# twosixlabs/csl-gan

Measured on AMD Instinct MI355X. Metric: images/sec/GPU CelebA DCResNet dp_mode=gc bs=128 at 1/2/4/8 MI355X, higher is better.
Workload: dtype f32; 1 GPU; CelebA DCResNet D-step: dp_mode=gc -gcm adaptive-pl -nms 32, WGAN-GP on mean samples, 3x64x64; compute_dtype=fp32_auto, storage_dtype=fp32, launch=hip_graph, batch_per_gpu=128, global_batch=128, parallelism=dp1, materialize=ghost, grad_sample_dtype=fp32, fuse_passes=True

## Files before the change

csl_gan_amd/csrc/igemm_x3.hip:

```cpp
#include <stdlib.h>
#include "common.h"
#include "igemm.h"

namespace cslgan {

typedef float f32x16 __attribute__((ext_vector_type(16)));
typedef float f32x2 __attribute__((ext_vector_type(2)));
typedef __bf16 bf16x2 __attribute__((ext_vector_type(2)));
typedef __bf16 bf16x8 __attribute__((ext_vector_type(8)));
typedef unsigned int u32x4 __attribute__((ext_vector_type(4)));

namespace {

constexpr unsigned XOOB = 0xFFFFFFF0u;
constexpr unsigned XFAR = 0xFFFF0000u;
constexpr int XH_MAX = 160;
constexpr int XROW = 12, XQROW = 6, XQIMG = 40;

__device__ __forceinline__ unsigned xpack(float lo, float hi) {
    const f32x2 v = {lo, hi};
    return __builtin_bit_cast(unsigned, __builtin_convertvector(v, bf16x2));
}
__device__ __forceinline__ float xlo(unsigned u) { return __uint_as_float(u << 16); }
__device__ __forceinline__ float xhi(unsigned u) { return __uint_as_float(u & 0xffff0000u); }
struct x3_t { uint2 hi, mid, lo; };
__device__ __forceinline__ x3_t xsplit4(const float4& v) {
    x3_t r;
    r.hi = make_uint2(xpack(v.x, v.y), xpack(v.z, v.w));
    const float r0 = v.x - xlo(r.hi.x), r1 = v.y - xhi(r.hi.x), r2 = v.z - xlo(r.hi.y), r3 = v.w - xhi(r.hi.y);
    r.mid = make_uint2(xpack(r0, r1), xpack(r2, r3));
    r.lo = make_uint2(xpack(r0 - xlo(r.mid.x), r1 - xhi(r.mid.x)), xpack(r2 - xlo(r.mid.y), r3 - xhi(r.mid.y)));
    return r;
}
__device__ __forceinline__ float4 xload4(__amdgpu_buffer_rsrc_t r, unsigned byte_off) {
    const u32x4 v = __builtin_amdgcn_raw_buffer_load_b128(r, (int)byte_off, 0, 0);
    return make_float4(__uint_as_float(v.x), __uint_as_float(v.y), __uint_as_float(v.z), __uint_as_float(v.w));
}

}

template <int BN, int NP, bool GEN, bool AFF = false>
__global__ __launch_bounds__(256, 2) void igemm_x3h_kernel(const KcParams p) {
    constexpr int BM = 128, TM = 2, TN = BN / 64;
    constexpr bool F32 = NP == 0;
    constexpr int NI = F32 ? 1 : NP;
    constexpr int NO = F32 ? 2 : NP;
    constexpr int PXU = F32 ? 4 : 2;
    constexpr int IMG = 2 * XH_MAX * PXU;
    __shared__ __attribute__((aligned(16))) uint4 Hs[2][NI][IMG];
    __shared__ int s_off[BM];
    __shared__ int s_roff[BM];

    const int tid = threadIdx.x;
    const int nwg = p.tiles_m * p.tiles_n;
    const int cs = p.csplit > 1 ? p.csplit : 1;
    const int wgs = xcd_remap(blockIdx.x, nwg * cs);
    const int split = cs > 1 ? wgs % cs : 0;
    const int wg = cs > 1 ? wgs / cs : wgs;
    const int tile_mg = wg / p.tiles_n, tile_n = wg - tile_mg * p.tiles_n;
    const bool accumulate = GEN && p.acc_classes;
    const int n_sub = accumulate ? p.n_cls : ((GEN && p.pair_mode) ? 2 : 1);
    const int lane = tid & 63, wid = tid >> 6;
    const int r = lane & 31, h = lane >> 5;
    const int wm = wid >> 1, wn = wid & 1;
    const int n0 = tile_n * BN;
    const __amdgpu_buffer_rsrc_t a_rsrc = __builtin_amdgcn_make_buffer_rsrc(const_cast<float*>(p.a), 0, p.a_bytes, 0x00020000);

    f32x16 acc[TM][TN];
#pragma unroll 1
    for (int sub = 0; sub < n_sub; ++sub) {
        int ci = 0, tile_in_cls;
        if (accumulate) {
            ci = sub;
            tile_in_cls = tile_mg;
        } else if (GEN && p.pair_mode) {
            const int pg = tile_mg / p.tiles_per_cls;
            ci = p.pair_cls[pg][sub];
            tile_in_cls = tile_mg - pg * p.tiles_per_cls;
        } else {
            if (GEN) {
#pragma unroll 1
                while (ci + 1 < p.n_cls && tile_mg >= p.cls[ci + 1].tile0) ++ci;
            }
            tile_in_cls = tile_mg - p.cls[ci].tile0;
        }
        const KcClass& kc = p.cls[ci];
        const int M = kc.M, OHc = kc.OHc, OWc = kc.OWc, T = kc.T;
        const int m0 = tile_in_cls * BM;
        const int HW_ = kc.halo_w, HH_ = kc.halo_h;
        const bool quad = GEN && kc.patch == 2;
        const int hpix_img = HH_ * HW_;
        const int hpix = quad ? 4 * hpix_img : hpix_img;
        const int img_stride = p.AH * p.AW * p.AC;
        const int ay_mul = (GEN && kc.ay_mul) ? kc.ay_mul : 1, ay_off = GEN ? kc.ay_off : 0;
        const int ax_mul = (GEN && kc.ax_mul) ? kc.ax_mul : 1, ax_off = GEN ? kc.ax_off : 0;
        const int nkw = kc.nkw;
        const int ystep = T > nkw ? (int)kc.ty[nkw] - (int)kc.ty[0] : 0;
        const int xstep = nkw > 1 ? (int)kc.tx[1] - (int)kc.tx[0] : 0;
        const int dy0 = (int)kc.ty[0] - kc.ty_min, dx0 = (int)kc.tx[0] - kc.tx_min;

        constexpr int HREG = (2 * XH_MAX * 4 + 255) / 256;
        unsigned h_goff[HREG];
        int h_lds[HREG];
        unsigned pp_mask = 0;
        int aff_off[2] = {0, 0};
        {
            int p_img[2], p_y0[2], p_x0[2];
            bool p_ok[2];
#pragma unroll
            for (int pp = 0; pp < 2; ++pp) {
                const int m = m0 + 64 * pp;
                p_ok[pp] = m < M;
                const RowCoord rc = kc_decode_row(p_ok[pp] ? m : 0, OHc, OWc, quad ? 0 : 1);
                p_img[pp] = rc.img * img_stride;
                if (AFF) aff_off[pp] = rc.img * p.AC + (tid & 3) * 4;
                p_y0[pp] = rc.oy + kc.ty_min;
                p_x0[pp] = rc.ox + kc.tx_min;
            }
            const int h_total = 2 * hpix * 4;
#pragma unroll
            for (int j = 0; j < HREG; ++j) {
                const int idx = tid + 256 * j;
                const int ch = idx & 3, pixg = idx >> 2;
                const int pp = pixg >= hpix ? 1 : 0;
                pp_mask |= (unsigned)pp << j;
                const int pix = pixg - pp * hpix;
                const int si = quad ? pix / hpix_img : 0;
                const int rem = pix - si * hpix_img;
                const int hy = rem / HW_, hx = rem - hy * HW_;
                const int iy = (p_y0[pp] + hy) * ay_mul + ay_off, ix = (p_x0[pp] + hx) * ax_mul + ax_off;
                const bool in_img = idx < h_total && p_ok[pp] && (unsigned)iy < (unsigned)p.VH && (unsigned)ix < (unsigned)p.VW;
                h_goff[j] = in_img ? 4u * (unsigned)(p_img[pp] + si * img_stride + (iy * p.AW + ix) * p.AC + ch * 4) : XFAR;
                const int lpx = quad ? si * XQIMG + hy * XQROW + hx : hy * XROW + hx;
                h_lds[j] = idx >= h_total ? -1 : (F32 ? (pp * XH_MAX + lpx) * 4 + (ch ^ ((hx + hy) & 3)) : (pp * XH_MAX + lpx) * 4 + (ch ^ ((hy & 1) << 1)));
            }
        }
        const int n_cc_all = p.AC >> 4;
        const int cc_lo = cs > 1 ? split * n_cc_all / cs : 0;
        const int n_cc = cs > 1 ? (split + 1) * n_cc_all / cs - cc_lo : n_cc_all;
        const float lo = (AFF && !p.in_relu) ? -__builtin_inff() : 0.f;
        float4 rh[HREG];
        float4 sc0, sc1, sh0, sh1;
        const __amdgpu_buffer_rsrc_t sc_rsrc = __builtin_amdgcn_make_buffer_rsrc(const_cast<float*>(AFF ? p.in_scale : p.a), 0, 0xFFFFFFF0u, 0x00020000);
        const __amdgpu_buffer_rsrc_t sh_rsrc = __builtin_amdgcn_make_buffer_rsrc(const_cast<float*>(AFF ? p.in_shift : p.a), 0, 0xFFFFFFF0u, 0x00020000);
        auto fetch_halo = [&](int cc) {
            const unsigned co = 64u * (unsigned)(cc + cc_lo);
#pragma unroll
            for (int j = 0; j < HREG; ++j) rh[j] = xload4(a_rsrc, h_goff[j] + co);
            if (AFF) {
                sc0 = xload4(sc_rsrc, 4u * (unsigned)aff_off[0] + co); sh0 = xload4(sh_rsrc, 4u * (unsigned)aff_off[0] + co);
                sc1 = xload4(sc_rsrc, 4u * (unsigned)aff_off[1] + co); sh1 = xload4(sh_rsrc, 4u * (unsigned)aff_off[1] + co);
            }
        };
        auto commit_halo = [&](int buf) {
#pragma unroll
            for (int j = 0; j < HREG; ++j) {
                if (AFF) {
                    const bool second = (pp_mask >> j) & 1u;
                    const float m = h_goff[j] != XFAR ? 1.f : 0.f;
                    rh[j].x = fmaxf(fmaf((second ? sc1.x : sc0.x) * m, rh[j].x, (second ? sh1.x : sh0.x) * m), lo);
                    rh[j].y = fmaxf(fmaf((second ? sc1.y : sc0.y) * m, rh[j].y, (second ? sh1.y : sh0.y) * m), lo);
                    rh[j].z = fmaxf(fmaf((second ? sc1.z : sc0.z) * m, rh[j].z, (second ? sh1.z : sh0.z) * m), lo);
                    rh[j].w = fmaxf(fmaf((second ? sc1.w : sc0.w) * m, rh[j].w, (second ? sh1.w : sh0.w) * m), lo);
                }
                if (h_lds[j] >= 0) {
                    uint2* img0 = reinterpret_cast<uint2*>(&Hs[buf][0][0]);
                    if (F32) {
                        Hs[buf][0][h_lds[j]] = make_uint4(__float_as_uint(rh[j].x), __float_as_uint(rh[j].y), __float_as_uint(rh[j].z), __float_as_uint(rh[j].w));
                    } else if (NP == 1) {
                        img0[h_lds[j]] = make_uint2(xpack(rh[j].x, rh[j].y), xpack(rh[j].z, rh[j].w));
                    } else {
                        const x3_t t3 = xsplit4(rh[j]);
                        img0[h_lds[j]] = t3.hi;
                        reinterpret_cast<uint2*>(&Hs[buf][NI > 1 ? 1 : 0][0])[h_lds[j]] = t3.mid;
                        reinterpret_cast<uint2*>(&Hs[buf][NI > 2 ? 2 : 0][0])[h_lds[j]] = t3.lo;
                    }
                }
            }
        };

        const unsigned piece_bytes = F32 ? 32u : 2u * (unsigned)p.Nn * (unsigned)kc.Kdim;
        const __amdgpu_buffer_rsrc_t w3_rsrc = __builtin_amdgcn_make_buffer_rsrc(
            const_cast<char*>(reinterpret_cast<const char*>(p.w3) + (F32 ? 4ll : 2ll * NP) * kc.w_off), 0,
            F32 ? 4u * (unsigned)p.Nn * (unsigned)kc.Kdim : NP * piece_bytes, 0x00020000);
        const unsigned n_bytes = F32 ? 64u : 32u;
        const unsigned step_bytes = n_bytes * (unsigned)p.Nn;
        unsigned b_off[TN];
#pragma unroll
        for (int j = 0; j < TN; ++j) {
            const int n = n0 + wn * TN * 32 + j * 32 + r;
            b_off[j] = n < p.Nn ? n_bytes * (unsigned)n + 16u * (unsigned)h : XOOB;
        }
        const int n_steps = n_cc * T;
        const unsigned step0_bytes = (unsigned)(cc_lo * T) * step_bytes;
        u32x4 B0[NO][TN], B1[NO][TN];
        auto load_b = [&](int step, u32x4 (&dst)[NO][TN]) {
            const unsigned kb = (unsigned)step * step_bytes + step0_bytes;
            const unsigned past = step >= n_steps ? XOOB : 0u;
#pragma unroll
            for (int j = 0; j < TN; ++j) {
                const unsigned bad = past | (b_off[j] == XOOB ? XOOB : 0u);
#pragma unroll
                for (int c = 0; c < NO; ++c)
                    dst[c][j] = __builtin_amdgcn_raw_buffer_load_b128(w3_rsrc, (int)((b_off[j] + kb + c * piece_bytes) | bad), 0, 0);
            }
        };

        int a_idx[TM];
        int a_rot[TM];
#pragma unroll
        for (int i = 0; i < TM; ++i) {
            const int qq = i * 32 + r;
            const int ly = quad ? (qq >> 2) & 3 : qq >> 3;
            const int lx = quad ? qq & 3 : qq & 7;
            const int lpix = quad ? (qq >> 4) * XQIMG + ly * XQROW + lx : ly * XROW + lx;
            a_idx[i] = F32 ? (wm * XH_MAX + lpix) * 4 : (wm * XH_MAX + lpix) * 2 + (h ^ (ly & 1));
            a_rot[i] = (lx + ly) & 3;
        }
        const int HWL = quad ? XQROW : XROW;
        u32x4 A0[NO][TM], A1[NO][TM];
        auto read_a = [&](int buf, int dy, int dx, u32x4 (&dst)[NO][TM]) {
            const int poff = dy * HWL + dx;
#pragma unroll
            for (int i = 0; i < TM; ++i) {
                if (F32) {
                    const int rot = (a_rot[i] + dy + dx) & 3, base = a_idx[i] + 4 * poff;
#pragma unroll
                    for (int c = 0; c < NO; ++c) {
                        const uint4 v = Hs[buf][0][base + ((2 * c + h) ^ rot)];
                        dst[c][i] = u32x4{v.x, v.y, v.z, v.w};
                    }
                } else {
                    const int at = (a_idx[i] + 2 * poff) ^ (dy & 1);
#pragma unroll
                    for (int c = 0; c < NO; ++c) {
                        const uint4 v = Hs[buf][c < NI ? c : 0][at];
                        dst[c][i] = u32x4{v.x, v.y, v.z, v.w};
                    }
                }
            }
        };

        if (!accumulate || sub == 0) {
#pragma unroll
            for (int i = 0; i < TM; ++i)
#pragma unroll
                for (int j = 0; j < TN; ++j)
#pragma unroll
                    for (int v = 0; v < 16; ++v) acc[i][j][v] = 0.f;
        }

        fetch_halo(0);
        load_b(0, B0);
        load_b(1, B1);
        commit_halo(0);
        __syncthreads();
        read_a(0, dy0, dx0, A0);

        int ti = 0, tj = 0, cc = 0;
        auto k_step = [&](int s, u32x4 (&b_cur)[NO][TN], u32x4 (&A)[NO][TM], u32x4 (&An)[NO][TM]) {
            int tjn = tj + 1, tin = ti;
            if (tjn == nkw) { tjn = 0; tin = ti + 1; }
            const int tn = tin * nkw + tjn;
            const bool last_tap = tn == T;
            const bool commit_now = tn == T - 1 || T == 1;
            if (last_tap) { tin = 0; tjn = 0; }
            const bool more_chunks = cc + 1 < n_cc;
            const int buf = cc & 1;
            const int rbuf = last_tap ? buf ^ 1 : buf;
            const int dyn = dy0 + tin * ystep, dxn = dx0 + tjn * xstep;
            if (ti == 0 && tj == 0 && more_chunks) fetch_halo(cc + 1);
#pragma unroll
            for (int i = 0; i < TM; ++i) {
#pragma unroll
                for (int j = 0; j < TN; ++j) {
                    f32x16 a = acc[i][j];
                    if constexpr (F32) {
#pragma unroll
                        for (int c = 0; c < 2; ++c) {
                            a = __builtin_amdgcn_mfma_f32_32x32x2f32(__uint_as_float(b_cur[c][j].x), __uint_as_float(A[c][i].x), a, 0, 0, 0);
                            a = __builtin_amdgcn_mfma_f32_32x32x2f32(__uint_as_float(b_cur[c][j].y), __uint_as_float(A[c][i].y), a, 0, 0, 0);
                            a = __builtin_amdgcn_mfma_f32_32x32x2f32(__uint_as_float(b_cur[c][j].z), __uint_as_float(A[c][i].z), a, 0, 0, 0);
                            a = __builtin_amdgcn_mfma_f32_32x32x2f32(__uint_as_float(b_cur[c][j].w), __uint_as_float(A[c][i].w), a, 0, 0, 0);
                        }
                    } else {
                        auto bf = [](const u32x4& v) { return __builtin_bit_cast(bf16x8, v); };
                        if (NP == 3) {
                            a = __builtin_amdgcn_mfma_f32_32x32x16_bf16(bf(b_cur[NO - 1][j]), bf(A[0][i]), a, 0, 0, 0);
                            a = __builtin_amdgcn_mfma_f32_32x32x16_bf16(bf(b_cur[0][j]), bf(A[NO - 1][i]), a, 0, 0, 0);
                            a = __builtin_amdgcn_mfma_f32_32x32x16_bf16(bf(b_cur[NO > 1 ? 1 : 0][j]), bf(A[NO > 1 ? 1 : 0][i]), a, 0, 0, 0);
                            a = __builtin_amdgcn_mfma_f32_32x32x16_bf16(bf(b_cur[NO > 1 ? 1 : 0][j]), bf(A[0][i]), a, 0, 0, 0);
                            a = __builtin_amdgcn_mfma_f32_32x32x16_bf16(bf(b_cur[0][j]), bf(A[NO > 1 ? 1 : 0][i]), a, 0, 0, 0);
                        }
                        a = __builtin_amdgcn_mfma_f32_32x32x16_bf16(bf(b_cur[0][j]), bf(A[0][i]), a, 0, 0, 0);
                    }
                    acc[i][j] = a;
                    if (i == 0 && j == 0) {
                        __builtin_amdgcn_sched_barrier(0);
                        read_a(rbuf, dyn, dxn, An);
                        __builtin_amdgcn_sched_barrier(0);
                    }
                }
            }
            load_b(s + 2, b_cur);
            if (commit_now && more_chunks) {
                commit_halo(buf ^ 1);
                __syncthreads();
            }
            if (last_tap) cc = cc + 1;
            ti = tin; tj = tjn;
        };
        {
            int s = 0;
#pragma unroll 1
            for (; s + 1 < n_steps; s += 2) {
                k_step(s, B0, A0, A1);
                k_step(s + 1, B1, A1, A0);
            }
            if (s < n_steps) k_step(s, B0, A0, A1);
        }
        __syncthreads();

        if (accumulate && sub + 1 < n_sub) continue;
        if (tid < BM) {
            const int m = m0 + tid;
            int off = -1, roff = 0;
            if (m < M) {
                const RowCoord rc = kc_decode_row(m, OHc, OWc, quad ? 0 : 1);
                off = kc_out_offset(p, kc, rc);
                if (p.res) roff = kc_res_offset(p, kc, rc);
            }
            s_off[tid] = off;
            s_roff[tid] = roff;
        }
        __syncthreads();
        const bool gn = !GEN && p.gn_part != nullptr;
        float4 gk[TN][4], g1[TN][4], g2[TN][4];
#pragma unroll
        for (int i = 0; i < TM; ++i) {
            const int row = wm * 64 + i * 32 + r;
            const int off = s_off[row], roff = s_roff[row];
            if (off < 0) continue;
#pragma unroll
            for (int j = 0; j < TN; ++j) {
#pragma unroll
                for (int q = 0; q < 4; ++q) {
                    const int n = n0 + wn * TN * 32 + j * 32 + 8 * q + 4 * h;
                    if (n >= p.Nn) continue;
                    float4 val = make_float4(acc[i][j][4 * q], acc[i][j][4 * q + 1], acc[i][j][4 * q + 2], acc[i][j][4 * q + 3]);
                    if (cs > 1) {
                        *reinterpret_cast<float4*>(p.part + (long long)split * p.out_floats + off + n) = val;
                        continue;
                    }
                    if (p.bias) {
                        const float4 bv = *reinterpret_cast<const float4*>(p.bias + n);
                        val.x += bv.x; val.y += bv.y; val.z += bv.z; val.w += bv.w;
                    }
                    if (p.res) {
                        const float4 rv = *reinterpret_cast<const float4*>(p.res + roff + n);
                        val.x += rv.x; val.y += rv.y; val.z += rv.z; val.w += rv.w;
                    }
                    if (gn) {
                        if (i == 0) {
                            const int src = lane & 32;
                            gk[j][q] = make_float4(__shfl(val.x, src), __shfl(val.y, src), __shfl(val.z, src), __shfl(val.w, src));
                            g1[j][q] = make_float4(0.f, 0.f, 0.f, 0.f);
                            g2[j][q] = make_float4(0.f, 0.f, 0.f, 0.f);
                        }
                        const float4 d = make_float4(val.x - gk[j][q].x, val.y - gk[j][q].y, val.z - gk[j][q].z, val.w - gk[j][q].w);
                        g1[j][q].x += d.x; g1[j][q].y += d.y; g1[j][q].z += d.z; g1[j][q].w += d.w;
                        g2[j][q].x = fmaf(d.x, d.x, g2[j][q].x); g2[j][q].y = fmaf(d.y, d.y, g2[j][q].y);
                        g2[j][q].z = fmaf(d.z, d.z, g2[j][q].z); g2[j][q].w = fmaf(d.w, d.w, g2[j][q].w);
                    }
                    if (p.act == CSLGAN_ACT_LRELU02) {
                        val.x = val.x > 0.f ? val.x : 0.2f * val.x; val.y = val.y > 0.f ? val.y : 0.2f * val.y;
                        val.z = val.z > 0.f ? val.z : 0.2f * val.z; val.w = val.w > 0.f ? val.w : 0.2f * val.w;
                    } else if (p.act == CSLGAN_ACT_RELU) {
                        val.x = val.x > 0.f ? val.x : 0.f; val.y = val.y > 0.f ? val.y : 0.f;
                        val.z = val.z > 0.f ? val.z : 0.f; val.w = val.w > 0.f ? val.w : 0.f;
                    } else if (p.act == CSLGAN_ACT_TANH) {
                        val.x = tanhf(val.x); val.y = tanhf(val.y); val.z = tanhf(val.z); val.w = tanhf(val.w);
                    }
                    if (p.mask) {
                        const float4 mv = *reinterpret_cast<const float4*>(p.mask + off + n);
                        val.x *= mv.x > 0.f ? 1.f : 0.2f; val.y *= mv.y > 0.f ? 1.f : 0.2f;
                        val.z *= mv.z > 0.f ? 1.f : 0.2f; val.w *= mv.w > 0.f ? 1.f : 0.2f;
                    }
                    *reinterpret_cast<float4*>(p.out + off + n) = val;
                }
            }
        }
        if (gn) {
            float* s_ch = reinterpret_cast<float*>(&Hs[0][0][0]);
            float* s_k = s_ch + 2 * BN * 2;
            const bool valid = s_off[wm * 64] >= 0;
            constexpr int NV = TN * 32;
            float v[NV];
#pragma unroll
            for (int j = 0; j < TN; ++j)
#pragma unroll
                for (int q = 0; q < 4; ++q) {
                    const float a1[4] = {g1[j][q].x, g1[j][q].y, g1[j][q].z, g1[j][q].w}, a2[4] = {g2[j][q].x, g2[j][q].y, g2[j][q].z, g2[j][q].w};
#pragma unroll
                    for (int e = 0; e < 4; ++e) { v[((j * 4 + q) * 4 + e) * 2] = a1[e]; v[((j * 4 + q) * 4 + e) * 2 + 1] = a2[e]; }
                }
#pragma unroll
            for (int s = 0; s < 5; ++s) {
                const int n = NV >> (s + 1), mask = 16 >> s;
                const bool up = (r & mask) != 0;
#pragma unroll
                for (int i = 0; i < n; ++i) {
                    const float keep = up ? v[n + i] : v[i], send = up ? v[i] : v[n + i];
                    v[i] = keep + __shfl_xor(send, mask);
                }
            }
            if (valid) {
                if (r == 0) {
#pragma unroll
                    for (int j = 0; j < TN; ++j)
#pragma unroll
                        for (int q = 0; q < 4; ++q)
                            *reinterpret_cast<float4*>(s_k + wm * BN + wn * TN * 32 + j * 32 + 8 * q + 4 * h) = gk[j][q];
                }
                if (NV == 64) {
                    const int cl = wn * TN * 32 + (r >> 4) * 32 + 8 * ((r >> 2) & 3) + 4 * h + (r & 3);
                    s_ch[(wm * BN + cl) * 2] = v[0];
                    s_ch[(wm * BN + cl) * 2 + 1] = v[1];
                } else {
                    const int cc = r >> 1, cl = wn * TN * 32 + 8 * (cc >> 2) + 4 * h + (cc & 3);
                    s_ch[(wm * BN + cl) * 2 + (r & 1)] = v[0];
                }
            }
            __syncthreads();
            const int cpg = p.gn_cpg, gpt = BN / cpg;
            if (tid < 2 * gpt) {
                const int pp = tid / gpt, gl = tid - pp * gpt;
                const int m = m0 + 64 * pp, c0 = n0 + gl * cpg;
                if (m < M && c0 < p.Nn) {
                    const float* q = s_ch + (pp * BN + gl * cpg) * 2;
                    const float* kq = s_k + pp * BN + gl * cpg;
                    float sum = 0.f;
                    for (int c = 0; c < cpg; ++c) sum += kq[c] + q[2 * c] * (1.f / 64.f);
                    const float mg = sum / (float)cpg;
                    float m2 = 0.f;
                    for (int c = 0; c < cpg; ++c) {
                        const float m1 = q[2 * c] * (1.f / 64.f), dm = kq[c] + m1 - mg;
                        float c2 = q[2 * c + 1] - q[2 * c] * m1;
                        m2 += (c2 < 0.f ? 0.f : c2) + 64.f * dm * dm;
                    }
                    const int per = OHc * OWc, img = m / per, slot = (m - img * per) >> 6;
                    float* o = p.gn_part + (((long long)img * p.gn_slots + slot) * (p.Nn / cpg) + c0 / cpg) * 2;
                    o[0] = mg * 64.f * (float)cpg;
                    o[1] = m2;
                }
            }
        }
        __syncthreads();
    }
}

__global__ __launch_bounds__(256) void x3h_split_reduce_kernel(const float* __restrict__ part, int cs, long long stride, float* __restrict__ out,
                                                               long long n4, int Nn, const float* __restrict__ bias,
                                                               const float* __restrict__ mask, int act) {
    for (long long i = (long long)blockIdx.x * 256 + threadIdx.x; i < n4; i += (long long)gridDim.x * 256) {
        float4 v = reinterpret_cast<const float4*>(part)[i];
        for (int s = 1; s < cs; ++s) {
            const float4 u = reinterpret_cast<const float4*>(part + s * stride)[i];
            v.x += u.x; v.y += u.y; v.z += u.z; v.w += u.w;
        }
        if (bias) {
            const float4 bv = *reinterpret_cast<const float4*>(bias + (int)((i << 2) % Nn));
            v.x += bv.x; v.y += bv.y; v.z += bv.z; v.w += bv.w;
        }
        if (act == CSLGAN_ACT_LRELU02) {
            v.x = v.x > 0.f ? v.x : 0.2f * v.x; v.y = v.y > 0.f ? v.y : 0.2f * v.y; v.z = v.z > 0.f ? v.z : 0.2f * v.z; v.w = v.w > 0.f ? v.w : 0.2f * v.w;
        } else if (act == CSLGAN_ACT_RELU) {
            v.x = v.x > 0.f ? v.x : 0.f; v.y = v.y > 0.f ? v.y : 0.f; v.z = v.z > 0.f ? v.z : 0.f; v.w = v.w > 0.f ? v.w : 0.f;
        } else if (act == CSLGAN_ACT_TANH) {
            v.x = tanhf(v.x); v.y = tanhf(v.y); v.z = tanhf(v.z); v.w = tanhf(v.w);
        }
        if (mask) {
            const float4 mv = reinterpret_cast<const float4*>(mask)[i];
            v.x *= mv.x > 0.f ? 1.f : 0.2f; v.y *= mv.y > 0.f ? 1.f : 0.2f; v.z *= mv.z > 0.f ? 1.f : 0.2f; v.w *= mv.w > 0.f ? 1.f : 0.2f;
        }
        reinterpret_cast<float4*>(out)[i] = v;
    }
}

template <int NP>
__global__ void split_filter_x3_kernel(const float* __restrict__ w, int Nn, int T, int C, unsigned short* __restrict__ w3) {
    const long long n_el = (long long)Nn * T * C, n4 = n_el >> 2;
    for (long long i = (long long)blockIdx.x * blockDim.x + threadIdx.x; i < n4; i += (long long)gridDim.x * blockDim.x) {
        const long long e = i << 2;
        const int c = (int)(e % C);
        const long long nt = e / C;
        const int t = (int)(nt % T), n = (int)(nt / T);
        const long long dst = ((((long long)(c >> 4) * T + t) * Nn + n) << 4) + (c & 15);
        if (NP == 0) {
            *reinterpret_cast<float4*>(reinterpret_cast<float*>(w3) + dst) = reinterpret_cast<const float4*>(w)[i];
            continue;
        }
        const x3_t s3 = xsplit4(reinterpret_cast<const float4*>(w)[i]);
        *reinterpret_cast<uint2*>(w3 + dst) = s3.hi;
        if (NP == 3) {
            *reinterpret_cast<uint2*>(w3 + n_el + dst) = s3.mid;
            *reinterpret_cast<uint2*>(w3 + 2 * n_el + dst) = s3.lo;
        }
    }
}

int split_filter_x3(const float* w, int Nn, int T, int C, void* w3, hipStream_t st, int pieces) {
    if (C % 16) return CSLGAN_OK;
    long long nb = ((long long)Nn * T * C / 4 + 255) / 256;
    nb = nb > 2048 ? 2048 : (nb < 1 ? 1 : nb);
    if (pieces == 0) hipLaunchKernelGGL(split_filter_x3_kernel<0>, dim3((unsigned)nb), dim3(256), 0, st, w, Nn, T, C, reinterpret_cast<unsigned short*>(w3));
    else if (pieces == 1) hipLaunchKernelGGL(split_filter_x3_kernel<1>, dim3((unsigned)nb), dim3(256), 0, st, w, Nn, T, C, reinterpret_cast<unsigned short*>(w3));
    else hipLaunchKernelGGL(split_filter_x3_kernel<3>, dim3((unsigned)nb), dim3(256), 0, st, w, Nn, T, C, reinterpret_cast<unsigned short*>(w3));
    return check_launch("split_filter_x3_kernel");
}

static void tap_range(const KcClass& k, int& ymin, int& ymax, int& xmin, int& xmax) {
    ymin = 127; ymax = -128; xmin = 127; xmax = -128;
    for (int t = 0; t < k.T; ++t) {
        ymin = k.ty[t] < ymin ? k.ty[t] : ymin; ymax = k.ty[t] > ymax ? k.ty[t] : ymax;
        xmin = k.tx[t] < xmin ? k.tx[t] : xmin; xmax = k.tx[t] > xmax ? k.tx[t] : xmax;
    }
}

static int affine_taps(const KcClass& k) {
    int nkw = 1;
    while (nkw < k.T && k.ty[nkw] == k.ty[0]) ++nkw;
    if (k.T % nkw) return 0;
    const int nkh = k.T / nkw;
    const int xs = nkw > 1 ? k.tx[1] - k.tx[0] : 0, ys = nkh > 1 ? k.ty[nkw] - k.ty[0] : 0;
    if ((nkw > 1 && xs != 1 && xs != -1) || (nkh > 1 && ys != 1 && ys != -1)) return 0;
    for (int t = 0; t < k.T; ++t)
        if (k.ty[t] != k.ty[0] + (t / nkw) * ys || k.tx[t] != k.tx[0] + (t % nkw) * xs) return 0;
    return nkw;
}

bool x3h_eligible(const KcParams& p) {
    static const int env = [] { const char* e = getenv("CSLGAN_X3_HALO"); return e ? atoi(e) : 1; }();
    static const int env32 = [] { const char* e = getenv("CSLGAN_F32_HALO"); return e ? atoi(e) : 1; }();
    if (!p.bf16 && !env32) return false;
    if (!env || !p.w3 || p.sy != 1 || p.sx != 1 || (p.AC & 15) || p.Nn < 64 || p.ksplit > 1 || !aligned16(p.a) || !aligned16(p.w3)) return false;
    if ((p.Nn & 3) || (p.ldo & 3) || !aligned16(p.out) || (p.bias && !aligned16(p.bias)) || (p.res && !aligned16(p.res)) || (p.mask && !aligned16(p.mask))) return false;
    static const int quad_min = [] { const char* e = getenv("CSLGAN_X3_QUAD_MIN"); return e ? atoi(e) : 2048; }();
    for (int c = 0; c < p.n_cls; ++c) {
        const KcClass& k = p.cls[c];
        const bool quad = k.OHc == 4 && k.OWc == 4;
        if (k.T < 2 || (k.M & 63) || (k.Kdim & 3) || (k.w_off & 7)) return false;
        if (quad && (k.M < quad_min || !p.bf16)) return false;
        if (!quad && ((k.OHc & 7) || (k.OWc & 7))) return false;
        if (!affine_taps(k)) return false;
        int ymin, ymax, xmin, xmax;
        tap_range(k, ymin, ymax, xmin, xmax);
        const int lim = quad ? 2 : 4;
        if (ymax - ymin > lim || xmax - xmin > lim) return false;
    }
    return true;
}

int launch_x3h(KcParams& p, hipStream_t st) {
    if (p.a_bytes >= XFAR) { set_error("igemm_x3h: input tensor of 4 GB"); return CSLGAN_ERR_INVALID_ARG; }
    int tm = 0;
    bool gen = p.acc_classes != 0 || p.n_cls > 1;
    for (int c = 0; c < p.n_cls; ++c) {
        KcClass& k = p.cls[c];
        int ymin, ymax, xmin, xmax;
        tap_range(k, ymin, ymax, xmin, xmax);
        const bool quad = k.OHc == 4 && k.OWc == 4;
        const int side = quad ? 4 : 8;
        k.ty_min = ymin; k.tx_min = xmin; k.halo_h = side + ymax - ymin; k.halo_w = side + xmax - xmin;
        k.patch = quad ? 2 : 1;
        k.nkw = affine_taps(k);
        k.tile0 = tm;
        tm += (k.M + 127) / 128;
        gen = gen || quad || k.ay_mul > 1 || k.ax_mul > 1;
    }
    if (p.gn_part && gen) { set_error("igemm_x3h: GroupNorm partials need a single-class stride-1 launch"); return CSLGAN_ERR_INVALID_ARG; }
    if (p.in_scale && (gen || p.bf16 == 1 || !p.in_shift || !aligned16(p.in_scale) || !aligned16(p.in_shift))) {
        set_error("igemm_x3h: the input affine map needs a single-class stride-1 launch in fp32 or three-piece arithmetic and 16-byte aligned tables");
        return CSLGAN_ERR_INVALID_ARG;
    }
    p.tiles_m = tm;
    p.ksplit = 1;
    p.pair_mode = 0;
    bool same_m = true, same_t = true;
    for (int c = 1; c < p.n_cls; ++c) { same_m = same_m && p.cls[c].M == p.cls[0].M; same_t = same_t && p.cls[c].T == p.cls[0].T; }
    bool wide = p.Nn > 64;
    if (p.acc_classes) p.tiles_m = (p.cls[0].M + 127) / 128;
    static const int pair_min = [] { const char* e = getenv("CSLGAN_X3_PAIR_MIN"); return e ? atoi(e) : 256; }();
    if (!p.acc_classes && p.n_cls == 4 && same_m && !same_t) {
        const int tpc = (p.cls[0].M + 127) / 128;
        const long long paired = 2ll * tpc * (wide ? (p.Nn + 127) / 128 : (p.Nn + 63) / 64);
        if (paired >= pair_min) {
            int o[4] = {0, 1, 2, 3};
            for (int i = 0; i < 4; ++i)
                for (int j = i + 1; j < 4; ++j)
                    if (p.cls[o[j]].T > p.cls[o[i]].T) { const int t = o[i]; o[i] = o[j]; o[j] = t; }
            p.pair_mode = 1;
            p.pair_cls[0][0] = o[0]; p.pair_cls[0][1] = o[3];
            p.pair_cls[1][0] = o[1]; p.pair_cls[1][1] = o[2];
            p.tiles_per_cls = tpc;
            p.tiles_m = 2 * tpc;
        }
    }
    static const int wide_min = [] { const char* e = getenv("CSLGAN_X3_WIDE_MIN"); return e ? atoi(e) : 192; }();
    if (wide && (long long)p.tiles_m * ((p.Nn + 127) / 128) < wide_min) wide = false;
    p.tiles_n = wide ? (p.Nn + 127) / 128 : (p.Nn + 63) / 64;
    p.csplit = 1;
    static const int split_env = [] { const char* e = getenv("CSLGAN_X3_SPLIT"); return e ? atoi(e) : 8; }();
    const long long tiles = (long long)p.tiles_m * p.tiles_n;
    if (split_env > 1 && p.part && !p.res && p.ldo == p.Nn && p.out_floats > 0 && (p.out_floats & 3) == 0 && aligned16(p.part) && tiles < 512) {
        const int n_cc = p.AC >> 4;
        double best = (double)((tiles + 255) / 256);
        for (int s = 2; s <= split_env && n_cc / s >= 2 && (long long)s * p.out_floats <= p.part_floats; ++s) {
            const double cost = (double)((tiles * s + 255) / 256) / s + 0.02 * s;
            if (cost < best - 1e-9) { best = cost; p.csplit = s; }
        }
    }
    const dim3 grid((unsigned)(tiles * p.csplit)), block(256);
    const bool x3 = p.bf16 == 3;
    if (p.csplit > 1)
        note_kernel(x3 ? "igemm_x3h_kernel<%d,3,%s,false>/s%d" : (p.bf16 ? "igemm_x3h_kernel<%d,1,%s,false>/s%d" : "igemm_x3h_kernel<%d,0,%s,false>/s%d"), wide ? 128 : 64,
                    gen ? "true" : "false", p.csplit);
    else if (p.in_scale)
        note_kernel(x3 ? "igemm_x3h_kernel<%d,3,false,true>" : "igemm_x3h_kernel<%d,0,false,true>", wide ? 128 : 64);
    else
        note_kernel(x3 ? "igemm_x3h_kernel<%d,3,%s,false>" : (p.bf16 ? "igemm_x3h_kernel<%d,1,%s,false>" : "igemm_x3h_kernel<%d,0,%s,false>"), wide ? 128 : 64, gen ? "true" : "false");
    if (p.in_scale) {
        if (x3 && wide) hipLaunchKernelGGL((igemm_x3h_kernel<128, 3, false, true>), grid, block, 0, st, p);
        else if (x3) hipLaunchKernelGGL((igemm_x3h_kernel<64, 3, false, true>), grid, block, 0, st, p);
        else if (wide) hipLaunchKernelGGL((igemm_x3h_kernel<128, 0, false, true>), grid, block, 0, st, p);
        else hipLaunchKernelGGL((igemm_x3h_kernel<64, 0, false, true>), grid, block, 0, st, p);
    } else if (!p.bf16) {
        if (wide && gen) hipLaunchKernelGGL((igemm_x3h_kernel<128, 0, true>), grid, block, 0, st, p);
        else if (wide) hipLaunchKernelGGL((igemm_x3h_kernel<128, 0, false>), grid, block, 0, st, p);
        else if (gen) hipLaunchKernelGGL((igemm_x3h_kernel<64, 0, true>), grid, block, 0, st, p);
        else hipLaunchKernelGGL((igemm_x3h_kernel<64, 0, false>), grid, block, 0, st, p);
    } else if (x3) {
        if (wide && gen) hipLaunchKernelGGL((igemm_x3h_kernel<128, 3, true>), grid, block, 0, st, p);
        else if (wide) hipLaunchKernelGGL((igemm_x3h_kernel<128, 3, false>), grid, block, 0, st, p);
        else if (gen) hipLaunchKernelGGL((igemm_x3h_kernel<64, 3, true>), grid, block, 0, st, p);
        else hipLaunchKernelGGL((igemm_x3h_kernel<64, 3, false>), grid, block, 0, st, p);
    } else {
        if (wide && gen) hipLaunchKernelGGL((igemm_x3h_kernel<128, 1, true>), grid, block, 0, st, p);
        else if (wide) hipLaunchKernelGGL((igemm_x3h_kernel<128, 1, false>), grid, block, 0, st, p);
        else if (gen) hipLaunchKernelGGL((igemm_x3h_kernel<64, 1, true>), grid, block, 0, st, p);
        else hipLaunchKernelGGL((igemm_x3h_kernel<64, 1, false>), grid, block, 0, st, p);
    }
    if (int rc = check_launch("igemm_x3h_kernel")) return rc;
    if (p.csplit > 1) {
        const long long n4 = p.out_floats >> 2;
        long long nb = (n4 + 255) / 256;
        nb = nb > 4096 ? 4096 : nb;
        hipLaunchKernelGGL(x3h_split_reduce_kernel, dim3((unsigned)nb), dim3(256), 0, st, p.part, p.csplit, p.out_floats, p.out, n4, p.Nn, p.bias, p.mask, p.act);
        return check_launch("x3h_split_reduce_kernel");
    }
    return CSLGAN_OK;
}

}
```

Baseline: 19930 images/sec.

## Add shared-halo window kernel for multi-class implicit GEMM with bf16 pieces

Adds a new implicit-GEMM kernel variant that loads one input halo window per 64-row tile into LDS, shared across all kernel-tap classes. Each wave computes 32 filters with 32x32x16 bf16 MFMAs, double-buffering the A fragments and B weights and prefetching the next channel chunk's halo while the current one is consumed. It is dispatched when the classes share geometry, M is a multiple of 64, the halo fits the register/LDS budget and there is no split, residual, mask, GN or input-scale path. The aim is to cut redundant global loads and per-class kernel overhead, at the cost of large dynamic LDS, which may limit occupancy, and an extra code path.

```diff
diff --git a/csl_gan_amd/csrc/igemm_x3.hip b/csl_gan_amd/csrc/igemm_x3.hip
--- a/csl_gan_amd/csrc/igemm_x3.hip
+++ b/csl_gan_amd/csrc/igemm_x3.hip
@@ -456,6 +456,247 @@
             }
         }
         __syncthreads();
+    }
+}
+
+constexpr int XW_HREG = 8;
+
+template <int BN, int NP>
+__global__ __launch_bounds__(256, 2) void igemm_x3h_window_kernel(const KcParams p, const int plane_px) {
+    static_assert(BN == 128 && (NP == 1 || NP == 3), "window form: four waves x 32 filters, bf16 pieces");
+    constexpr int TM = 2;
+    extern __shared__ __attribute__((aligned(16))) uint4 Hw[];
+    __shared__ int s_off[64];
+
+    const int tid = threadIdx.x;
+    const int wg = xcd_remap(blockIdx.x, p.tiles_m * p.tiles_n);
+    const int tile_m = wg / p.tiles_n, tile_n = wg - tile_m * p.tiles_n;
+    const int lane = tid & 63, wn = tid >> 6;
+    const int r = lane & 31, h = lane >> 5;
+    const int n0 = tile_n * BN, m0 = tile_m * 64;
+    const int n_cls = p.n_cls;
+    const int OHc = p.cls[0].OHc, OWc = p.cls[0].OWc;
+    const bool quad = p.cls[0].patch == 2;
+    const int HWL = quad ? XQROW : XROW;
+    const int pimg = n_cls * plane_px * 2;
+    const __amdgpu_buffer_rsrc_t a_rsrc = __builtin_amdgcn_make_buffer_rsrc(const_cast<float*>(p.a), 0, p.a_bytes, 0x00020000);
+
+    int c_T[IG_MAX_CLS], c_nkw[IG_MAX_CLS], c_dy0[IG_MAX_CLS], c_dx0[IG_MAX_CLS], c_ys[IG_MAX_CLS], c_xs[IG_MAX_CLS], cum[IG_MAX_CLS + 1];
+    unsigned c_wb[IG_MAX_CLS], c_pb[IG_MAX_CLS];
+    int t_tot = 0;
+    cum[0] = 0;
+#pragma unroll
+    for (int c = 0; c < IG_MAX_CLS; ++c) {
+        const KcClass& kc = p.cls[c];
+        const bool on = c < n_cls;
+        c_T[c] = on ? kc.T : 0;
+        c_nkw[c] = on ? kc.nkw : 1;
+        c_ys[c] = kc.T > kc.nkw ? (int)kc.ty[kc.nkw] - (int)kc.ty[0] : 0;
+        c_xs[c] = kc.nkw > 1 ? (int)kc.tx[1] - (int)kc.tx[0] : 0;
+        c_dy0[c] = (int)kc.ty[0] - kc.ty_min;
+        c_dx0[c] = (int)kc.tx[0] - kc.tx_min;
+        c_wb[c] = 2u * NP * (unsigned)kc.w_off;
+        c_pb[c] = 2u * (unsigned)p.Nn * (unsigned)kc.Kdim;
+        t_tot += c_T[c];
+        cum[c + 1] = cum[c] + (on ? (quad ? 4 : 1) * kc.halo_h * kc.halo_w : 0);
+    }
+    auto sel = [](const auto (&v)[IG_MAX_CLS], int c) { return c == 0 ? v[0] : (c == 1 ? v[1] : (c == 2 ? v[2] : v[3])); };
+
+    unsigned h_goff[XW_HREG];
+    int h_lds[XW_HREG];
+    {
+        const RowCoord rc = kc_decode_row(m0, OHc, OWc, quad ? 0 : 1);
+        const int img_stride = p.AH * p.AW * p.AC;
+        const int p_img = rc.img * img_stride;
+        const int h_total = cum[IG_MAX_CLS] * 4;
+#pragma unroll
+        for (int j = 0; j < XW_HREG; ++j) {
+            const int idx = tid + 256 * j;
+            const int ch = idx & 3, pixg = idx >> 2;
+            int cl = 0, base = 0, hw = p.cls[0].halo_w, hh = p.cls[0].halo_h, ymin = p.cls[0].ty_min, xmin = p.cls[0].tx_min;
+            int aym = p.cls[0].ay_mul, ayo = p.cls[0].ay_off, axm = p.cls[0].ax_mul, axo = p.cls[0].ax_off;
+#pragma unroll
+            for (int c = 1; c < IG_MAX_CLS; ++c) {
+                const KcClass& kc = p.cls[c];
+                if (c < n_cls && pixg >= cum[c]) {
+                    cl = c; base = cum[c]; hw = kc.halo_w; hh = kc.halo_h; ymin = kc.ty_min; xmin = kc.tx_min;
+                    aym = kc.ay_mul; ayo = kc.ay_off; axm = kc.ax_mul; axo = kc.ax_off;
+                }
+            }
+            const int pix = pixg - base;
+            const int hpix_img = hh * hw;
+            const int si = quad ? pix / hpix_img : 0;
+            const int rem = pix - si * hpix_img;
+            const int hy = rem / hw, hx = rem - hy * hw;
+            const int iy = (rc.oy + ymin + hy) * (aym ? aym : 1) + ayo, ix = (rc.ox + xmin + hx) * (axm ? axm : 1) + axo;
+            const bool in_img = idx < h_total && (unsigned)iy < (unsigned)p.VH && (unsigned)ix < (unsigned)p.VW;
+            h_goff[j] = in_img ? 4u * (unsigned)(p_img + si * img_stride + (iy * p.AW + ix) * p.AC + ch * 4) : XFAR;
+            const int lpx = cl * plane_px + (quad ? si * XQIMG + hy * XQROW + hx : hy * XROW + hx);
+            h_lds[j] = idx >= h_total ? -1 : lpx * 4 + (ch ^ ((hy & 1) << 1));
+        }
+    }
+    const int n_cc = p.AC >> 4;
+    float4 rh[XW_HREG];
+    auto fetch_halo = [&](int cc) {
+        const unsigned co = 64u * (unsigned)cc;
+#pragma unroll
+        for (int j = 0; j < XW_HREG; ++j) rh[j] = xload4(a_rsrc, h_goff[j] + co);
+    };
+    auto commit_halo = [&]() {
+        uint2* img0 = reinterpret_cast<uint2*>(Hw);
+#pragma unroll
+        for (int j = 0; j < XW_HREG; ++j) {
+            if (h_lds[j] >= 0) {
+                if (NP == 1) {
+                    img0[h_lds[j]] = make_uint2(xpack(rh[j].x, rh[j].y), xpack(rh[j].z, rh[j].w));
+                } else {
+                    const x3_t t3 = xsplit4(rh[j]);
+                    img0[h_lds[j]] = t3.hi;
+                    img0[2 * pimg + h_lds[j]] = t3.mid;
+                    img0[4 * pimg + h_lds[j]] = t3.lo;
+                }
+            }
+        }
+    };
+
+    const unsigned step_bytes = 32u * (unsigned)p.Nn;
+    const __amdgpu_buffer_rsrc_t w3_rsrc = __builtin_amdgcn_make_buffer_rsrc(const_cast<void*>(p.w3), 0,
+                                                                              2u * NP * (unsigned)p.Nn * (unsigned)p.AC * (unsigned)t_tot, 0x00020000);
+    const int nb = n0 + wn * 32 + r;
+    const unsigned b_off = nb < p.Nn ? 32u * (unsigned)nb + 16u * (unsigned)h : XOOB;
+    u32x4 B0[NP], B1[NP];
+    int fci = 0, ft = 0, fcc = 0;
+    auto load_b = [&](u32x4 (&dst)[NP]) {
+        const int tf = sel(c_T, fci);
+        const unsigned kb = sel(c_wb, fci) + (unsigned)(fcc * tf + ft) * step_bytes;
+        const unsigned pb = sel(c_pb, fci);
+        const unsigned bad = (fcc >= n_cc ? XOOB : 0u) | (b_off == XOOB ? XOOB : 0u);
+#pragma unroll
+        for (int c = 0; c < NP; ++c) dst[c] = __builtin_amdgcn_raw_buffer_load_b128(w3_rsrc, (int)((b_off + kb + c * pb) | bad), 0, 0);
+        const bool cls_end = ft + 1 == tf;
+        ft = cls_end ? 0 : ft + 1;
+        const int fn = fci + (cls_end ? 1 : 0);
+        const bool chunk_end = fn == n_cls;
+        fci = chunk_end ? 0 : fn;
+        fcc += chunk_end ? 1 : 0;
+    };
+
+    int a_idx[TM];
+#pragma unroll
+    for (int i = 0; i < TM; ++i) {
+        const int qq = i * 32 + r;
+        const int ly = quad ? (qq >> 2) & 3 : qq >> 3;
+        const int lx = quad ? qq & 3 : qq & 7;
+        const int lpix = quad ? (qq >> 4) * XQIMG + ly * XQROW + lx : ly * XROW + lx;
+        a_idx[i] = lpix * 2 + (h ^ (ly & 1));
+    }
+    u32x4 A0[NP][TM], A1[NP][TM];
+    auto read_a = [&](int cls, int dy, int dx, u32x4 (&dst)[NP][TM]) {
+        const int poff = cls * plane_px + dy * HWL + dx;
+#pragma unroll
+        for (int i = 0; i < TM; ++i) {
+            const int at = (a_idx[i] + 2 * poff) ^ (dy & 1);
+#pragma unroll
+            for (int c = 0; c < NP; ++c) {
+                const uint4 v = Hw[c * pimg + at];
+                dst[c][i] = u32x4{v.x, v.y, v.z, v.w};
+            }
+        }
+    };
+
+    f32x16 acc[TM];
+#pragma unroll
+    for (int i = 0; i < TM; ++i)
+#pragma unroll
+        for (int v = 0; v < 16; ++v) acc[i][v] = 0.f;
+
+    fetch_halo(0);
+    load_b(B0);
+    load_b(B1);
+    commit_halo();
+    __syncthreads();
+    read_a(0, c_dy0[0], c_dx0[0], A0);
+
+    int ci = 0, ti = 0, tj = 0, g = 0, cc = 0;
+    auto k_step = [&](u32x4 (&b_cur)[NP], u32x4 (&A)[NP][TM], u32x4 (&An)[NP][TM]) {
+        const int nkw = sel(c_nkw, ci);
+        int tjn = tj + 1, tin = ti, cin = ci, gn = g + 1;
+        if (tjn == nkw) { tjn = 0; tin = ti + 1; }
+        if (tin * nkw + tjn == sel(c_T, ci)) { tin = 0; tjn = 0; cin = ci + 1; }
+        const bool last_tap = gn == t_tot;
+        if (last_tap) { cin = 0; gn = 0; }
+        const bool commit_now = gn == t_tot - 1;
+        const bool more_chunks = cc + 1 < n_cc;
+        const int dyn = sel(c_dy0, cin) + tin * sel(c_ys, cin), dxn = sel(c_dx0, cin) + tjn * sel(c_xs, cin);
+        if (g == 0 && more_chunks) fetch_halo(cc + 1);
+#pragma unroll
+        for (int i = 0; i < TM; ++i) {
+            f32x16 a = acc[i];
+            auto bf = [](const u32x4& v) { return __builtin_bit_cast(bf16x8, v); };
+            if (NP == 3) {
+                a = __builtin_amdgcn_mfma_f32_32x32x16_bf16(bf(b_cur[NP - 1]), bf(A[0][i]), a, 0, 0, 0);
+                a = __builtin_amdgcn_mfma_f32_32x32x16_bf16(bf(b_cur[0]), bf(A[NP - 1][i]), a, 0, 0, 0);
+                a = __builtin_amdgcn_mfma_f32_32x32x16_bf16(bf(b_cur[NP > 1 ? 1 : 0]), bf(A[NP > 1 ? 1 : 0][i]), a, 0, 0, 0);
+                a = __builtin_amdgcn_mfma_f32_32x32x16_bf16(bf(b_cur[NP > 1 ? 1 : 0]), bf(A[0][i]), a, 0, 0, 0);
+                a = __builtin_amdgcn_mfma_f32_32x32x16_bf16(bf(b_cur[0]), bf(A[NP > 1 ? 1 : 0][i]), a, 0, 0, 0);
+            }
+            a = __builtin_amdgcn_mfma_f32_32x32x16_bf16(bf(b_cur[0]), bf(A[0][i]), a, 0, 0, 0);
+            acc[i] = a;
+            if (i == 0) {
+                __builtin_amdgcn_sched_barrier(0);
+                read_a(cin, dyn, dxn, An);
+                __builtin_amdgcn_sched_barrier(0);
+            }
+        }
+        load_b(b_cur);
+        if (commit_now && more_chunks) {
+            __syncthreads();
+            commit_halo();
+            __syncthreads();
+        }
+        if (last_tap) cc = cc + 1;
+        ci = cin; ti = tin; tj = tjn; g = gn;
+    };
+    {
+        const int n_steps = n_cc * t_tot;
+        int s = 0;
+#pragma unroll 1
+        for (; s + 1 < n_steps; s += 2) {
+            k_step(B0, A0, A1);
+            k_step(B1, A1, A0);
+        }
+        if (s < n_steps) k_step(B0, A0, A1);
+    }
+
+    if (tid < 64) {
+        const int m = m0 + tid;
+        s_off[tid] = m < p.cls[0].M ? kc_out_offset(p, p.cls[0], kc_decode_row(m, OHc, OWc, quad ? 0 : 1)) : -1;
+    }
+    __syncthreads();
+#pragma unroll
+    for (int i = 0; i < TM; ++i) {
+        const int off = s_off[i * 32 + r];
+        if (off < 0) continue;
+#pragma unroll
+        for (int q = 0; q < 4; ++q) {
+            const int n = n0 + wn * 32 + 8 * q + 4 * h;
+            if (n >= p.Nn) continue;
+            float4 val = make_float4(acc[i][4 * q], acc[i][4 * q + 1], acc[i][4 * q + 2], acc[i][4 * q + 3]);
+            if (p.bias) {
+                const float4 bv = *reinterpret_cast<const float4*>(p.bias + n);
+                val.x += bv.x; val.y += bv.y; val.z += bv.z; val.w += bv.w;
+            }
+            if (p.act == CSLGAN_ACT_LRELU02) {
+                val.x = val.x > 0.f ? val.x : 0.2f * val.x; val.y = val.y > 0.f ? val.y : 0.2f * val.y;
+                val.z = val.z > 0.f ? val.z : 0.2f * val.z; val.w = val.w > 0.f ? val.w : 0.2f * val.w;
+            } else if (p.act == CSLGAN_ACT_RELU) {
+                val.x = val.x > 0.f ? val.x : 0.f; val.y = val.y > 0.f ? val.y : 0.f;
+                val.z = val.z > 0.f ? val.z : 0.f; val.w = val.w > 0.f ? val.w : 0.f;
+            } else if (p.act == CSLGAN_ACT_TANH) {
+                val.x = tanhf(val.x); val.y = tanhf(val.y); val.z = tanhf(val.z); val.w = tanhf(val.w);
+            }
+            *reinterpret_cast<float4*>(p.out + off + n) = val;
+        }
     }
 }
 
@@ -620,8 +861,32 @@
             if (cost < best - 1e-9) { best = cost; p.csplit = s; }
         }
     }
+    const bool x3 = p.bf16 == 3;
+    const char* win_env = getenv("CSLGAN_X3_WINDOW");
+    if (p.acc_classes && p.bf16 && p.csplit == 1 && !p.res && !p.mask && !p.gn_part && !p.in_scale && (!win_env || atoi(win_env) != 0)) {
+        bool same = true;
+        int hh_max = 0, px = 0;
+        const bool quad = p.cls[0].patch == 2;
+        for (int c = 0; c < p.n_cls; ++c) {
+            const KcClass& k = p.cls[c];
+            same = same && k.M == p.cls[0].M && k.OHc == p.cls[0].OHc && k.OWc == p.cls[0].OWc && k.patch == p.cls[0].patch && k.oy0 == p.cls[0].oy0 &&
+                   k.ox0 == p.cls[0].ox0;
+            hh_max = k.halo_h > hh_max ? k.halo_h : hh_max;
+            px += (quad ? 4 : 1) * k.halo_h * k.halo_w;
+        }
+        const int plane_px = quad ? XH_MAX : hh_max * XROW;
+        if (same && (p.cls[0].M & 63) == 0 && px * 4 <= XW_HREG * 256 && plane_px <= XH_MAX) {
+            p.tiles_m = p.cls[0].M / 64;
+            p.tiles_n = (p.Nn + 127) / 128;
+            const unsigned lds = (unsigned)(x3 ? 3 : 1) * (unsigned)p.n_cls * (unsigned)plane_px * 32u;
+            const dim3 wgrid((unsigned)((long long)p.tiles_m * p.tiles_n));
+            note_kernel(x3 ? "igemm_x3h_kernel<128,3,true,false>[window]" : "igemm_x3h_kernel<128,1,true,false>[window]");
+            if (x3) hipLaunchKernelGGL((igemm_x3h_window_kernel<128, 3>), wgrid, dim3(256), lds, st, p, plane_px);
+            else hipLaunchKernelGGL((igemm_x3h_window_kernel<128, 1>), wgrid, dim3(256), lds, st, p, plane_px);
+            return check_launch("igemm_x3h_window_kernel");
+        }
+    }
     const dim3 grid((unsigned)(tiles * p.csplit)), block(256);
-    const bool x3 = p.bf16 == 3;
     if (p.csplit > 1)
         note_kernel(x3 ? "igemm_x3h_kernel<%d,3,%s,false>/s%d" : (p.bf16 ? "igemm_x3h_kernel<%d,1,%s,false>/s%d" : "igemm_x3h_kernel<%d,0,%s,false>/s%d"), wide ? 128 : 64,
                     gen ? "true" : "false", p.csplit);
```

Result: slower. 18630 images/sec, median of 2 (-6.5%).
